# ppjian19/PhoreGen

Hardware: AMD Instinct MI355X
Metric: denoise-steps/sec (batch=128, ~40-atom graphs) (higher is better)
Workload: dtype f32; 1 GPU; BASELINE.json configs[2]: ONE batch of 128 LigPhore-shaped graphs (n~N(40,6) atoms, p~N(107,30) pharmacophore nodes), partitioned over 1 GPU(s) by the fitted step cost, steps t=999.. of the 1000-step sampler, device Philox noise, trajectory written; graphs_total=128, graphs_rank0=128, n_ctx=18401, n_lig=5115, e_knn=588832, e_bond=203720, e3=8087028, parallelism=graph-sharded x1, final RCCL gather only, triplet_workgroups_rank0=256

## Files before the change

include/phoregen_hip.h:

```cpp
#ifndef PHOREGEN_HIP_H
#define PHOREGEN_HIP_H

#include <stdint.h>

#ifdef __cplusplus
extern "C" {
#endif

const char* pg_last_error(void);
int pg_abi_version(void);
int pg_abi_struct_sizes(int* out, int n);

int pg_order_point_create(void** ev);
int pg_order_point_destroy(void* ev);
int pg_order_point_record(void* ev, void* stream);
int pg_order_point_wait(void* ev, void* stream);
int pg_debug_order_point_fence_free(int on);

enum {
  PG_OP_RECORD = 0, PG_OP_WAIT = 1, PG_OP_GEMM = 2, PG_OP_SEG_ATTN = 3, PG_OP_EMBED_CTX = 4, PG_OP_EMBED_BOND = 5, PG_OP_KNN_CTX = 6,
  PG_OP_LIG_NORMALS = 7, PG_OP_EDGE_GATE = 8, PG_OP_KNN_GROUP_BY_KIND = 9, PG_OP_BOND_SMEAR = 10, PG_OP_ATTN_FOLD_QUERY = 11,
  PG_OP_ATTN_UNFOLD_VALUE = 12, PG_OP_APPLY_DX = 13, PG_OP_LAYER_GEOM = 14, PG_OP_ROWS_LINEAR = 15, PG_OP_ATOM_COUNT = 16
};
#define PG_PROGRAM_LANES 4
#define PG_LAUNCH_MAX_ARGS 12
typedef struct {
  int32_t op;
  int32_t lane;
  int32_t ev;
  int32_t n_arg;
  uint64_t a[PG_LAUNCH_MAX_ARGS];
} PgLaunch;
int pg_program_create(const PgLaunch* list, int n, int n_events, void** prog);
int pg_program_run(void* prog, void* const* streams );
int pg_program_length(void* prog);
int pg_program_destroy(void* prog);

int pg_micro_mfma_f32(int workgroups, int iters, float* sink, double* flops, void* stream);

int pg_selftest_mfma(int* d_result, void* stream);
int pg_selftest_philox(const uint32_t* ctr_key, int n, uint32_t* out, void* stream);
int pg_debug_force_generic_seg(int mask);

typedef struct {
  const float* X;   int ldx;  int K1;
  const float* X2;  int ldx2; int K2;
  const float* W;   int ldw;
  const float* bias;
  const float* ln_gamma; const float* ln_beta;
  const float* add1; int ld_add1; const int* idx1;
  const float* add2; int ld_add2; const int* idx2;
  float out_scale;
  int   act;
  float* Y; int ldy; int M; int N;
  const int* rows;
  int add_rows;
} PgGemm;
int pg_gemm(const PgGemm* p, void* stream);
int pg_debug_gemm_streaming(int on);

typedef struct {
  int n_graphs, n_ctx, n_lig, n_phore, n_bond;
  int max_nlig;
  int max_gctx;
  const int* g_ctx_off;
  const int* g_nph;
  const int* g_nlig;
  const int* g_eid_off;
  const int* eid;
  const int* ctx_graph;
  const uint8_t* ctx_is_lig;
  const int* lig2ctx;
  const int* bond_src;
  const int* bond_dst;
  const int* bond_desc;
  const int* g_bond_off;
  const int* edge_ref;
} PgTopo;

int pg_embed_ctx(const PgTopo* t, const float* h_node_pert , const float* pos_pert ,
                 const int64_t* time_step , const float* W_node ,
                 const float* t_offset , const float* t_coeff ,
                 const float* h_phore_emb , const float* pos_phore ,
                 const int* phore2ctx , float* h_ctx , float* x_ctx ,
                 void* stream);
int pg_embed_bond(const PgTopo* t, const float* h_edge_pert , const int* bond_graph,
                  const int64_t* time_step, const float* W_edge , const float* t_offset,
                  const float* t_coeff, float* h_bond , void* stream);

// ... 187 lines not shown
```

phoregen_amd/csrc/gemm.hip:

```cpp
#include <stdlib.h>

#include "common.h"
#include "../../include/phoregen_hip.h"

namespace pg {

constexpr int BM = 128, BN = 128, BK = 32, LDT = BK + 1;


__global__ __launch_bounds__(256) void gemm_kernel(PgGemm p PG_ABL_PARAM) {
  __shared__ __attribute__((aligned(16))) float smem[(BM + BN) * LDT];
  float* const As = smem;
  float* const Bs = smem + BM * LDT;
  __shared__ float rstat[BM * 2];

  const int tid = threadIdx.x, lane = tid & 63, wave = tid >> 6;
  const int col0 = blockIdx.x * BN;
  const int K = p.K1 + p.K2;
  for (int rb = blockIdx.y; rb * BM < p.M; rb += gridDim.y) {
  const int row0 = rb * BM;
  const int wr = (wave >> 1) * 64, wc = (wave & 1) * 64;
  const bool ln = p.ln_gamma != nullptr;

  if (ln) {
// ... 187 lines not shown
  const float bias = (b && m < n_out) ? b[m] : 0.f;
  const int n_tiles = (M + 63) >> 6;
  for (int tile = blockIdx.x; tile < n_tiles; tile += gridDim.x) {
    const int row0 = tile * 64;
    __syncthreads();
#pragma unroll
    for (int i = 0; i < 8; ++i) {
      const int r = (tid >> 5) + 8 * i, c4 = tid & 31;
      int grow = row0 + r;
      grow = grow < M ? grow : M - 1;
      const int src = rows ? rows[grow] : grow;
      *reinterpret_cast<f4*>(xs + r * RL_LD + 4 * c4) = __builtin_nontemporal_load(reinterpret_cast<const f4*>(X + (size_t)src * ldx) + c4);
    }
    __syncthreads();
    f4 acc = {bias, bias, bias, bias};
    const float* xa = xs + (16 * wave + m) * RL_LD + g;
#pragma unroll
    for (int s_ = 0; s_ < 32; ++s_) acc = mfma16(xa[4 * s_], wr[s_], acc);
    if (m < n_out) {
#pragma unroll
      for (int r = 0; r < 4; ++r) {
        const int grow = row0 + 16 * wave + 4 * g + r;
        if (grow < M) Y[(size_t)grow * ldy + m] = acc[r];
      }
    }
  }
}

}

namespace pg {
bool gemm_stream_eligible(const PgGemm* p);
int launch_gemm_stream(const PgGemm* p, hipStream_t st);
}

static int g_gemm_stream = 1;
extern "C" int pg_debug_gemm_streaming(int on) { const int old = g_gemm_stream; g_gemm_stream = on; return old; }

extern "C" int pg_gemm(const PgGemm* p, void* stream) {
  if (!p || !p->X || !p->W || !p->Y || p->M < 0 || p->N <= 0) { pg::set_error("pg_gemm: bad arguments"); return PG_ERR_ARG; }
  if (p->M == 0) return PG_OK;
  if (p->K2 > 0 && !p->X2) { pg::set_error("pg_gemm: K2 > 0 without X2"); return PG_ERR_ARG; }
  if (p->ln_gamma && (p->K2 != 0 || p->K1 != 128 || (p->ldx & 3) || ((size_t)p->X & 15))) { pg::set_error("pg_gemm: LayerNorm-on-load needs K1 == 128, K2 == 0, 16-byte aligned rows"); return PG_ERR_ARG; }
  if (g_gemm_stream && pg::gemm_stream_eligible(p)) return pg::launch_gemm_stream(p, (hipStream_t)stream);
  const int row_blocks = (p->M + pg::BM - 1) / pg::BM;
  dim3 grid((p->N + pg::BN - 1) / pg::BN, row_blocks < 65535 ? row_blocks : 65535);
  hipLaunchKernelGGL(pg::gemm_kernel, grid, dim3(256), 0, (hipStream_t)stream, *p PG_ABL_ARG("PG_GEMM_ABLATE"));
  return pg::check_launch("pg_gemm");
}

extern "C" int pg_rows_linear(const float* X, int ldx, int K, const float* W, const float* b, int n_out, int M,
                              const int* rows, float* Y, int ldy, void* stream) {
  if (n_out > 16 || n_out <= 0 || K <= 0 || K > 256) { pg::set_error("pg_rows_linear: n_out must be 1..16, K 1..256"); return PG_ERR_ARG; }
  if (M == 0) return PG_OK;
  if (K == 128 && (ldx & 3) == 0 && ((size_t)X & 15) == 0) {
    int blocks = (M + 63) / 64;
    if (blocks > 8 * kNumCU) blocks = 8 * kNumCU;
    hipLaunchKernelGGL(pg::rows_linear_mfma_kernel, dim3(blocks), dim3(256), 0, (hipStream_t)stream, X, ldx, W, b, n_out, M, rows, Y, ldy);
    return pg::check_launch("pg_rows_linear");
  }
  hipLaunchKernelGGL(pg::rows_linear_kernel, dim3((M + 3) / 4), dim3(256), 0, (hipStream_t)stream, X, ldx, K, W, b,
                     n_out, M, rows, Y, ldy);
  return pg::check_launch("pg_rows_linear");
}
```

phoregen_amd/engine.py:

```python
import ctypes as C

import torch

from . import hip, options
from .packing import HEAD_SCALE, ModelPack


_SIDE_STREAMS = {}


_TRI_GRID_CACHE = {}


def side_streams(device_index, stream_set=0):
    key = (device_index, stream_set)
    if key not in _SIDE_STREAMS:
        with torch.cuda.device(device_index):
            _SIDE_STREAMS[key] = [torch.cuda.Stream(), torch.cuda.Stream(), torch.cuda.Stream()]
    return _SIDE_STREAMS[key]


def _f(*shape, device, zero=False):
    return (torch.zeros if zero else torch.empty)(*shape, dtype=torch.float32, device=device)

# ... 2 lines not shown
    __slots__ = ('kind', '__name__', 'ops', 'start', 'lane', 'tensors')

    def __init__(self, kind, name, ops=None, start=None, lane=0, tensors=()):
        self.kind, self.__name__, self.ops, self.start, self.lane, self.tensors = kind, name, ops, start, lane, tensors

    @property
    def name(self):
        return self.__name__


class Engine:
    def __init__(self, pack: ModelPack, plan, knn_k=32, full=True, phore_only=False):
        self.lib = hip.lib()
        self.pack, self.plan, self.k = pack, plan, knn_k
        self.dev = plan.device
        self._keep = []
        self.debug = None
        self.timers = None
        self.trace = None
        self.tri_calls = []
        o = options.snapshot()
        self.multi_stream = o['streams']
        self.layer_ahead = o['layer_ahead']
        self.tri_split, self.tri_split_from = o['tri_split'], o['tri_split_from']
        self.tri_overlap = o['tri_overlap']
        self.chain_q_from = o['chain_q_from']
        self.tune_grid = o['tune_grid']
        self.tuned_tri_grid = None
        self.geom_split = o['geom_split'] == 'always' or (o['geom_split'] == 'auto' and self.plan.n_bond < o['geom_split_below'])
        self.ahead_v2 = o['ahead_v2'] == 'always' or (o['ahead_v2'] == 'auto' and self.plan.n_bond < o['ahead_v2_below'])
        self.step_ahead = o['step_ahead']
        self.pos_tiled, self.pos_tiled_below = o['pos_tiled'], o['pos_tiled_below']
        self.tri_grid = o['tri_grid']
        self._lane = 0
        self._n_points = 0
        self._points = {}
        self.c_program = o['c_program']
        self._compiled = {}
        self._side = None
        self.stream_set = 0
        self._alloc()
        if full:
            self.prog_phore = self._build_phore_program()
            if not phore_only:
                self.prog_fwd = self._build_forward_program()
                self.prog_step = self.prog_ahead = None

    def _alloc(self):
        p, d = self.plan, self.dev
        n, E, k = p.n_ctx, p.n_bond, self.k
        w = self.ws = type('WS', (), {})()
        w.in_h_node, w.in_pos = _f(p.n_lig, 12, device=d), _f(p.n_lig, 3, device=d)
        w.in_h_edge = _f(E, 6, device=d)
        w.in_t = torch.zeros(p.n_graphs, dtype=torch.int64, device=d)
        w.in_t_next = torch.zeros(p.n_graphs, dtype=torch.int64, device=d)
        w.h_phore_ctx, w.x_phore_ctx = _f(n, 18, device=d, zero=True), _f(n, 3, device=d, zero=True)
        w.pos_phore, w.phore_norm = _f(p.n_phore, 3, device=d), _f(p.n_phore, 3, device=d)
        w.nrm_phore_ctx = _f(n, 3, device=d, zero=True)
        w.is_ex = torch.zeros(p.n_phore, dtype=torch.uint8, device=d)
        w.hp_ctx, w.Yp = _f(n, 128, device=d), _f(n, 640, device=d)
        w.enc_ctx = _f(n, 128, device=d, zero=True)
        w.hp_emb = _f(p.n_phore, 128, device=d)
        w.cnt_hid = _f(n, 256, device=d)
        w.s_all, w.s_l = _f(p.n_phore, device=d), _f(p.n_phore, device=d)
        w.count_l, w.count_u = _f(p.n_graphs, device=d), _f(p.n_graphs, device=d)
        w.h = [_f(n, 128, device=d), _f(n, 128, device=d)]
        w.h_in = _f(n, 128, device=d)
        w.x = [_f(n, 3, device=d), _f(n, 3, device=d)]
        w.hb = [_f(E, 128, device=d), _f(E, 128, device=d)]
        w.nbr = torch.zeros(n, k, dtype=torch.int32, device=d)
        w.deg = torch.zeros(n, dtype=torch.int32, device=d)
        w.ew, w.nrm, w.G = _f(n, k, device=d), _f(n, 3, device=d), _f(E, 20, device=d)
        w.Y1, w.Y2 = _f(n, 1920, device=d), _f(n, 1280, device=d)
        w.Y1b = None
        w.q = [_f(n, 128, device=d) for _ in range(4)]
        w.U, w.S = [_f(n, 2048, device=d) for _ in range(3)], [_f(n, 2048, device=d) for _ in range(3)]
        w.swn = [_f(n, 16, device=d) for _ in range(3)]
        w.aggE, w.aggB = _f(n, 128, device=d, zero=True), _f(n, 128, device=d, zero=True)
        w.lin_tmp = _f(n, 128, device=d)
        w.CsB, w.P = _f(E, 256, device=d), _f(E, 256, device=d)
        w.CsB2 = _f(E, 256, device=d)
        w.Qd = _f(E, 256, device=d)
        w.qhid, w.qT = _f(E, 128, device=d), _f(E, 128, device=d)
        w.dxe, w.dxb = _f(n, 3, device=d, zero=True), _f(n, 3, device=d, zero=True)
        w.head = _f(n, 128, device=d)
        w.head_b = _f(E, 128, device=d)
        w.out_v, w.out_bond = _f(p.n_lig, 12, device=d), _f(E, 6, device=d)

    def _call(self, prog, fn, *args):
        assert len(args) + 1 == len(fn.argtypes), (fn.__name__, len(args) + 1, len(fn.argtypes))
        prog.append((fn, args, self._lane if self.multi_stream else 0))

    def _new_point(self):
        self._n_points += 1
        return self._n_points - 1

    def _order(self, prog, name, ops):
        if self.multi_stream and ops:
            prog.append((_Tap('order', name, ops=ops), None, -1))

    def _fork(self, prog, lanes):
        if not self.multi_stream:
            return
        pt = self._new_point()
        self._order(prog, 'fork', [('record', pt, 0)] + [('wait', pt, l) for l in lanes])

    def _join(self, prog, lanes):
        self._sync(prog, 0, lanes, name='join')

    def _sync(self, prog, waiter, on, name='sync'):
        if not self.multi_stream:
            return
        ops = []
        for l in on:
            pt = self._new_point()
            ops += [('record', pt, l), ('wait', pt, waiter)]
# ... 11 lines not shown
            return
        self._order(prog, 'wait', [('wait', pt, waiter)])

    def _event(self, prog, name, start):
        prog.append((_Tap('event', name, start=start, lane=self._lane if self.multi_stream else 0), None, -1))

    def _mark(self, prog, name, *tensors, lane=0):
        prog.append((_Tap('mark', name, tensors=tensors, lane=lane if self.multi_stream else 0), None, -1))

    def _tap(self, tap, streams):
        if tap.kind == 'order':
            for what, pt, lane in tap.ops:
                ev = self._points.get(pt)
                if ev is None:
                    ev = self._points[pt] = hip.OrderPoint()
                if what == 'record':
                    ev.record(streams[lane])
                else:
                    ev.wait(streams[lane])
        elif tap.kind == 'event':
            if self.timers is not None:
                ev = torch.cuda.Event(enable_timing=True)
                ev.record(streams[tap.lane])
                self.timers.setdefault(tap.name, []).append((tap.start, ev))
        elif self.debug is not None:
            with torch.cuda.stream(streams[tap.lane]):
                self.debug[tap.name] = tuple(t.clone() for t in tap.tensors)

    def kernel_ms(self, name):
        evs = self.timers.get(name, [])
        return [a.elapsed_time(b) for (sa, a), (sb, b) in zip(evs[0::2], evs[1::2]) if sa and not sb]

    def _gemm(self, prog, X, K1, W, Y, M, N, bias=None, X2=None, K2=0, ln=None, add1=None, idx1=None, add2=None,
              idx2=None, scale=1.0, act=hip.ACT_NONE, rows=None):
        g = hip.PgGemm()
        g.X, g.ldx, g.K1 = X.data_ptr(), X.stride(0), K1
        g.X2, g.ldx2, g.K2 = (X2.data_ptr(), X2.stride(0), K2) if X2 is not None else (None, 0, 0)
        g.W, g.ldw = W.data_ptr(), W.stride(0)
        g.bias = hip.ptr(bias)
        g.ln_gamma, g.ln_beta = (ln[0].data_ptr(), ln[1].data_ptr()) if ln is not None else (None, None)
        g.add1, g.ld_add1, g.idx1 = (add1.data_ptr(), add1.stride(0), hip.ptr(idx1)) if add1 is not None else (None, 0, None)
        g.add2, g.ld_add2, g.idx2 = (add2.data_ptr(), add2.stride(0), hip.ptr(idx2)) if add2 is not None else (None, 0, None)
        g.out_scale, g.act = scale, act
        g.Y, g.ldy, g.M, g.N = Y.data_ptr(), Y.stride(0), M, N
        g.rows = hip.ptr(rows)
        g.add_rows = add1.size(0) if add1 is not None else 0
        self._keep += [g, X, W, Y, bias, X2, ln, add1, idx1, add2, idx2, rows]
        self._call(prog, self.lib.pg_gemm, C.byref(g))

    def _seg(self, prog, mode, n_seg, seg_ids, a, **kw):
        s = hip.PgSegAttn()
        s.mode, s.n_seg, s.seg_ids = mode, n_seg, hip.ptr(seg_ids)
        s.knn_k = self.k
        s.ln_gk, s.ln_bk, s.ln_gv, s.ln_bv = (t.data_ptr() for t in (a.ln_gk, a.ln_bk, a.ln_gv, a.ln_bv))
        for key, val in kw.items():
            setattr(s, key, val.data_ptr() if torch.is_tensor(val) else val)
            self._keep.append(val)
        self._keep += [s, seg_ids, a]
        self._call(prog, self.lib.pg_seg_attn, self.plan.topo_ref, C.byref(s))

    def _query_gemm(self, prog, a, Y, col0, h_dst_lists, buf):
        n, wq = self.plan.n_ctx, self.ws.q[buf]
        qh = Y[:, col0 + 4 * 128: col0 + 5 * 128]
        self._gemm(prog, qh, 128, a.W2q, wq, n, 128, bias=a.b2q, ln=(a.q_ln_g, a.q_ln_b), scale=HEAD_SCALE)

    def _node_attention(self, prog, mode, a, Y, col0, x, h_dst_lists, out=None, dx=None, csrc=None, buf=0, extra=None,
                        query_done=False, qbuf=None):
        w, p, n = self.ws, self.plan, self.plan.n_ctx
        wq, wU, wS, wsw = w.q[buf if qbuf is None else qbuf], w.U[buf], w.S[buf], w.swn[buf]
        blk = lambda b: Y[:, col0 + 128 * b: col0 + 128 * (b + 1)]
        if not query_done:
            self._query_gemm(prog, a, Y, col0, h_dst_lists, buf)
        knn = mode in (hip.SEG_KNN_NODE, hip.SEG_KNN_POS)
        pos = mode in (hip.SEG_KNN_POS, hip.SEG_BOND_POS)
        fused = mode != hip.SEG_PHORE
        merged = knn and len(h_dst_lists) == 2 and all(n > 0 for _, n, _ in h_dst_lists)
        lists = [h_dst_lists[0]] if merged else h_dst_lists
        for seg_ids, n_seg, is_lig in lists:
            if not fused:
                self._call(prog, self.lib.pg_attn_fold_query, wq.data_ptr(), 128, a.W2k_l.data_ptr(), n_seg,
                           seg_ids.data_ptr(), wU.data_ptr())
            kw = dict(x=x, Cdst_k=blk(0), Cdst_v=blk(1), ld_cdst=Y.stride(0), U=wU)
            if knn:
                kw.update(nrm=w.nrm, nbr=w.nbr, deg=w.deg, ew=w.ew, Csrc_k=blk(2), Csrc_v=blk(3), ld_csrc=Y.stride(0),
                          Wf_k=a.Wf_k[is_lig], Wf_v=a.Wf_v[is_lig])
                if merged:
                    ids2, n2, lig2 = h_dst_lists[1]
                    kw.update(seg_ids2=ids2, n_seg2=n2, Wf_k2=a.Wf_k[lig2], Wf_v2=a.Wf_v[lig2])
            elif mode == hip.SEG_PHORE:
                kw.update(Csrc_k=blk(2), Csrc_v=blk(3), ld_csrc=Y.stride(0), Wf_k=a.Wf_k, Wf_v=a.Wf_v)
            else:
                kw.update(Csrc_k=csrc[:, 0:128], Csrc_v=csrc[:, 128:256], ld_csrc=csrc.stride(0))
            if pos:
                kw.update(W2xv_l=a.W2xv_l, b2xv=a.b2xv, dx=dx, accumulate_dx=0)
                tiled = self.pos_tiled == 'always' or (self.pos_tiled == 'auto' and n_seg <= self.pos_tiled_below)
                if tiled:
                    kw.update(pos_tiled=1)
            else:
                kw.update(S=wS, swn=wsw)
            if fused:
                kw.update(q=wq, W2k_l=a.W2k_l)
                if not pos:
# ... 77 lines not shown
        lig = [(p.lig2ctx, p.n_lig, True)]
        both = [(p.lig2ctx, p.n_lig, True), (p.phore2ctx, p.n_phore, False)]
        L0 = pk.layers[0]
        self._sync(prog, 3, (2,))
        self._lane = 3
        self._embed_bond(prog, w.in_t_next)
        hb_done = self._record(prog, 3)
        self._lane = 2
        self._embed_ctx(prog, w.in_t_next, coords=False)
        self._first_layer_gemm(prog, L0, w.h_in, w.Y1)
        y1_done = self._record(prog, 2)
        self._query_gemm(prog, L0.NE, w.Y1, 0, both, 3)
        self._wait(prog, 2, hb_done)
        self._triplet_queries(prog, L0, w.hb[0], w.Y1)
        self._lane = 3
        self._wait(prog, 3, y1_done)
        self._bond_node_rows(prog, L0, w.hb[0], w.Y1)
        self._node_attention(prog, hip.SEG_BOND_NODE, L0.NB, w.Y1, 5 * 128, w.x[0], lig, out=w.aggB, csrc=w.CsB2, buf=2)
        self._lane = 0
        return prog

    def pipelined_programs(self):
        if not (self.step_ahead and self.multi_stream and self.layer_ahead and self.plan.n_tri_iters):
            return None
        if self.prog_step is None:
            tri_calls, self.tri_calls = self.tri_calls, []
            self.prog_step = self._build_forward_program(step_ahead=True)
            self.step_tri_calls, self.tri_calls = self.tri_calls, tri_calls
            self.prog_ahead = self._build_ahead_program()
        return self.prog_step, self.prog_ahead

    def _first_layer_gemm(self, prog, L, h_in, Y1):
        p, n = self.plan, self.plan.n_ctx
        self._gemm(prog, h_in, 128, L.W_node1, Y1, n, 1920, bias=L.b_node1)

    def _triplet_queries(self, prog, L, hb_in, Y1):
        w, p, E = self.ws, self.plan, self.plan.n_bond
        self._gemm(prog, hb_in, 128, L.TB.W_q_hb, w.qhid, E, 128, add1=Y1[:, 14 * 128:15 * 128], idx1=p.bond_dst)
        self._gemm(prog, w.qhid, 128, L.TB.W2q, w.qT, E, 128, bias=L.TB.b2q, ln=(L.TB.q_ln_g, L.TB.q_ln_b), scale=HEAD_SCALE)

    def _bond_node_rows(self, prog, L, hb_in, Y1):
        w, p, E = self.ws, self.plan, self.plan.n_bond
        self._gemm(prog, hb_in, 128, L.NB.W_hb, w.CsB2, E, 256, add1=Y1[:, 7 * 128:9 * 128], idx1=p.bond_src)

    def _denoiser_program(self, prog, lig, both, heads=None, pre_join=None, step_ahead=False):
        w, p, pk, lib = self.ws, self.plan, self.pack, self.lib
        n, E, t = p.n_ctx, p.n_bond, p.topo_ref
        h, x, hb = w.h, w.x, w.hb
        g = pk.gate
        self._fork(prog, (1,))
        self._lane = 1
        self._call(prog, lib.pg_knn_ctx, t, x[0].data_ptr(), self.k, w.nbr.data_ptr(), w.deg.data_ptr())
        self._call(prog, lib.pg_edge_gate, t, x[0].data_ptr(), w.nbr.data_ptr(), w.deg.data_ptr(), self.k,
                   g['W0'].data_ptr(), g['b0'].data_ptr(), g['g'].data_ptr(), g['b'].data_ptr(), g['W3'].data_ptr(),
                   C.c_float(g['b3']), w.ew.data_ptr())
        self._mark(prog, 'graph', w.nbr, w.deg, w.ew, lane=1)
        self._call(prog, lib.pg_knn_group_by_kind, t, self.k, w.nbr.data_ptr(), w.deg.data_ptr(), w.ew.data_ptr())
        self._lane = 0
        cur = 0
        staged = bool(p.n_tri_iters)
        n_layers = len(pk.layers)
        ahead = self.layer_ahead and self.multi_stream
        v2 = self.ahead_v2 and ahead
        chain_q = self.multi_stream and (v2 or E >= self.chain_q_from)
        tri_grid = self.tri_grid if self.tri_grid >= 0 else ((192 if E < 15000 else 224 if E < 80000 else 0) if self.multi_stream else 0)
        self._tune = None
        if (self.tune_grid and self.tri_grid < 0 and self.multi_stream and staged and 0 < tri_grid <= 224):
            self._tune = dict(cands=[g for g in (tri_grid, tri_grid + 32, tri_grid - 32) if 128 <= g <= 256])

        if v2 and w.Y1b is None:
            w.Y1b = torch.empty_like(w.Y1)
        split = v2 and self.geom_split
# ... 79 lines not shown
            self._event(prog, 'triplet', False)
            if last:
                self._fork(prog, (3,))
                self._lane = 3
                heads[0](hbn)
            self._lane = 3 if v2 else 2
            if not pre:
                bond_node_rows(L, hbc, Y1c)
                self._node_attention(prog, hip.SEG_BOND_NODE, L.NB, Y1c, 5 * 128, xc, lig, out=w.aggB, csrc=w.CsB2, buf=1)
                if v2:
                    bn_done = self._record(prog, 3)
            self._lane = 1
            if not pre:
                self._query_gemm(prog, L.NE, Y1c, 0, both, 0)
            if pre0:
                self._sync(prog, 1, (2,))
            elif pre and v2:
                self._wait(prog, 1, ne_done)
            self._event(prog, 'knn_node', True)
            self._node_attention(prog, hip.SEG_KNN_NODE, L.NE, Y1c, 0, xc1, both, out=w.aggE, buf=0, query_done=True,
                                 qbuf=3 if pre else None)
            self._event(prog, 'knn_node', False)
            if pre0:
                self._sync(prog, 1, (3,))
            elif pre or v2:
                self._wait(prog, 1, bn_done)
            else:
                self._sync(prog, 1, (2,))
            self._gemm(prog, w.aggE, 128, L.W_lin2[:, :128], w.lin_tmp, n, 128, bias=L.b_lin, add1=hc)
            self._gemm(prog, w.aggB, 128, L.W_lin2[:, 128:], hn, n, 128, add1=w.lin_tmp)
            self._mark(prog, f'A{li}', w.aggE, w.aggB, lane=1)
            if early:
                hn_done = self._record(prog, 1)
            self._gemm(prog, hn, 128, L.W_node2, w.Y2, n, 1280, bias=L.b_node2)
            if v2:
                self._query_gemm(prog, L.PB, w.Y2, 5 * 128, lig, 1)
            more_ahead = ahead and li + 1 < n_layers and not last
            self._sync(prog, 0, (1,))
            if v2 and more_ahead:
                self._lane = 1
                first_layer_gemm(pk.layers[li + 1], hn, Y1n)
                y1_done = self._record(prog, 1)
            qlane = 2 if last else 3
            if early:
                self._wait(prog, 2, hn_done)
                self._lane = 2
                heads[1](hn)
                if not v2:
                    self._fork(prog, (2,))
            else:
                self._fork(prog, (2, 3) if (ahead and li + 1 < n_layers) else (qlane,))
            self._lane = qlane
            if not v2:
                self._query_gemm(prog, L.PB, w.Y2, 5 * 128, lig, 1)
                q_done = self._record(prog, qlane)
            if last and not early:
                heads[1](hn)
            elif ahead and li + 1 < n_layers:
                Ln = pk.layers[li + 1]
                self._lane = 2
                if v2:
                    self._wait(prog, 2, y1_done)
                else:
                    first_layer_gemm(Ln, hn, Y1n)
                    y1_done = self._record(prog, 2)
                triplet_queries(Ln, hbn, Y1n)
                if not v2:
# ... 270 lines not shown
```

phoregen_amd/hip.py:

```python
import ctypes as C
import struct
import sys
import os

import torch

_HERE = os.path.dirname(os.path.abspath(__file__))
LIB_PATH = os.path.join(_HERE, '_lib', 'libphoregen_hip.so')

c_fp = C.c_void_p
c_ip = C.c_void_p


class PgGemm(C.Structure):
    _fields_ = [('X', c_fp), ('ldx', C.c_int), ('K1', C.c_int),
                ('X2', c_fp), ('ldx2', C.c_int), ('K2', C.c_int),
                ('W', c_fp), ('ldw', C.c_int),
                ('bias', c_fp),
                ('ln_gamma', c_fp), ('ln_beta', c_fp),
                ('add1', c_fp), ('ld_add1', C.c_int), ('idx1', c_ip),
                ('add2', c_fp), ('ld_add2', C.c_int), ('idx2', c_ip),
                ('out_scale', C.c_float), ('act', C.c_int),
                ('Y', c_fp), ('ldy', C.c_int), ('M', C.c_int), ('N', C.c_int), ('rows', c_ip), ('add_rows', C.c_int)]


class PgTopo(C.Structure):
    _fields_ = [('n_graphs', C.c_int), ('n_ctx', C.c_int), ('n_lig', C.c_int), ('n_phore', C.c_int),
                ('n_bond', C.c_int), ('max_nlig', C.c_int), ('max_gctx', C.c_int),
                ('g_ctx_off', c_ip), ('g_nph', c_ip), ('g_nlig', c_ip), ('g_eid_off', c_ip), ('eid', c_ip),
                ('ctx_graph', c_ip), ('ctx_is_lig', c_ip), ('lig2ctx', c_ip), ('bond_src', c_ip),
                ('bond_dst', c_ip), ('bond_desc', c_ip), ('g_bond_off', c_ip), ('edge_ref', c_ip)]


class PgSegAttn(C.Structure):
    _fields_ = [('mode', C.c_int), ('n_seg', C.c_int), ('seg_ids', c_ip), ('seg_chunks', c_ip),
                ('x', c_fp), ('nrm', c_fp), ('nbr', c_ip), ('deg', c_ip), ('ew', c_fp), ('knn_k', C.c_int),
                ('Csrc_k', c_fp), ('Csrc_v', c_fp), ('ld_csrc', C.c_int),
                ('Cdst_k', c_fp), ('Cdst_v', c_fp), ('ld_cdst', C.c_int),
                ('Wf_k', c_fp), ('Wf_v', c_fp), ('Wg2_k', c_fp), ('Wg2_v', c_fp), ('G', c_fp),
                ('ln_gk', c_fp), ('ln_bk', c_fp), ('ln_gv', c_fp), ('ln_bv', c_fp),
                ('U', c_fp), ('q', c_fp), ('W2k_l', c_fp), ('W2v_l', c_fp), ('b2v', c_fp),
                ('W2xv_l', c_fp), ('b2xv', c_fp),
                ('S', c_fp), ('swn', c_fp), ('resid', c_fp), ('out', c_fp), ('dx', c_fp),
                ('accumulate_dx', C.c_int), ('alpha', c_fp), ('alpha_rows', C.c_int), ('efeat', c_fp), ('efeat_off', c_ip),
                ('tri_iters', c_ip), ('n_tri_iters', C.c_int), ('tri_counter', c_ip),
                ('seg_ids2', c_ip), ('n_seg2', C.c_int), ('Wf_k2', c_fp), ('Wf_v2', c_fp), ('tri_grid', C.c_int), ('pos_tiled', C.c_int), ('tri_max_nlig', C.c_int)]


class PgSegAttnGrad(C.Structure):
    _fields_ = [('gS', c_fp), ('gswn', c_fp), ('gdx', c_fp), ('gU', c_fp),
                ('gCdst_k', c_fp), ('gCdst_v', c_fp), ('ld_gcdst', C.c_int),
                ('gCsrc_k', c_fp), ('gCsrc_v', c_fp), ('ld_gcsrc', C.c_int),
                ('gWf_k', c_fp), ('gWf_v', c_fp), ('gbk', c_fp), ('gbv', c_fp),
                ('gW2xv_l', c_fp), ('gb2xv', c_fp), ('gx', c_fp), ('gnrm', c_fp), ('gew', c_fp),
                ('alpha', c_fp), ('alpha_rows', C.c_int), ('S', c_fp), ('swn', c_fp),
                ('rowbuf', c_fp), ('rowbuf_rows', C.c_int), ('grid', C.c_int), ('atom_order', c_ip),
# ... 220 lines not shown
```

phoregen_amd/options.py:

```python
import contextlib
import os

DEFAULTS = dict(
    streams=True,
    layer_ahead=True,
    ahead_v2='auto',
    ahead_v2_below=82000,
    pos_tiled='auto',
    pos_tiled_below=1500,
    step_ahead=True,
    c_program=True,
    geom_split='auto',
    geom_split_below=16000,
    tune_grid=True,
    chain_q_from=150000,
    tri_split=True,
    tri_split_from=82000,
    tri_overlap=3,
    tri_grid=-1,
    dgrad_mm=True,
    rows_sum=True,
    tri_onepass=True,
    wide_gemm=True,
    bwd_atom_sort=True,
    bwd_split='all',
    bwd_grid=256,
    tri_bwd_form=2,
    tri_bwd_grid=256,
    ph_onepass=True,
)

_tri = lambda v: {'0': 'never', '1': 'auto', '2': 'always'}[v]
_flag = lambda v: v != '0'
_ENV = {
    'PG_STREAMS': ('streams', _flag),
    'PG_LAYER_AHEAD': ('layer_ahead', _flag), 'PG_AHEAD_V2': ('ahead_v2', _tri), 'PG_AHEAD_V2_BELOW': ('ahead_v2_below', int), 'PG_TRI_GRID': ('tri_grid', int), 'PG_POS_TILED': ('pos_tiled', _tri), 'PG_POS_TILED_BELOW': ('pos_tiled_below', int), 'PG_C_PROGRAM': ('c_program', _flag), 'PG_STEP_AHEAD': ('step_ahead', _flag), 'PG_CHAIN_Q_FROM': ('chain_q_from', int), 'PG_TRI_SPLIT': ('tri_split', _flag), 'PG_TUNE_GRID': ('tune_grid', _flag), 'PG_GEOM_SPLIT': ('geom_split', _tri),
    'PG_DGRAD_MM': ('dgrad_mm', _flag),
    'PG_ROWS_SUM': ('rows_sum', _flag), 'PG_TRI_ONEPASS': ('tri_onepass', _flag), 'PG_WIDE_GEMM': ('wide_gemm', _flag), 'PG_BWD_GRID': ('bwd_grid', int), 'PG_BWD_SPLIT': ('bwd_split', lambda v: {'0': 'none', '1': 'knn', '2': 'all'}[v]), 'PG_BWD_ATOM_SORT': ('bwd_atom_sort', _flag),
    'PG_TRI_BWD_FORM': ('tri_bwd_form', int), 'PG_TRI_BWD_GRID': ('tri_bwd_grid', int), 'PG_PH_ONEPASS': ('ph_onepass', _flag),
}
_overrides = {}


def get(name):
    if name in _overrides:
        return _overrides[name]
    if os.environ.get('PHOREGEN_DEBUG') == '1':
        for var, (key, conv) in _ENV.items():
            if key == name and var in os.environ:
                return conv(os.environ[var])
    return DEFAULTS[name]


def snapshot():
    return {k: get(k) for k in DEFAULTS}


@contextlib.contextmanager
def override(**kw):
    unknown = set(kw) - set(DEFAULTS)
    if unknown:
        raise KeyError(f'phoregen_amd.options: unknown switch(es) {sorted(unknown)}')
    old = dict(_overrides)
    _overrides.update(kw)
    try:
        yield
    finally:
        _overrides.clear()
        _overrides.update(old)
# ... 1 lines not shown
```

Before: 54.51 steps/s.

## Fuse attention query LayerNorm and projection into the wide node GEMM

```diff
diff --git a/include/phoregen_hip.h b/include/phoregen_hip.h
--- a/include/phoregen_hip.h
+++ b/include/phoregen_hip.h
@@ -41,6 +41,15 @@
 int pg_selftest_mfma(int* d_result, void* stream);
 int pg_selftest_philox(const uint32_t* ctr_key, int n, uint32_t* out, void* stream);
 int pg_debug_force_generic_seg(int mask);
+
+typedef struct {
+  int col0;
+  const float* ln_gamma; const float* ln_beta;
+  const float* W2; int ldw2; const float* b2;
+  float scale;
+  float* Q; int ldq;
+} PgGemmTail;
+#define PG_GEMM_MAX_TAILS 2
 
 typedef struct {
   const float* X;   int ldx;  int K1;
@@ -55,6 +64,8 @@
   float* Y; int ldy; int M; int N;
   const int* rows;
   int add_rows;
+  int n_tail;
+  PgGemmTail tail[PG_GEMM_MAX_TAILS];
 } PgGemm;
 int pg_gemm(const PgGemm* p, void* stream);
 int pg_debug_gemm_streaming(int on);
diff --git a/phoregen_amd/csrc/gemm.hip b/phoregen_amd/csrc/gemm.hip
--- a/phoregen_amd/csrc/gemm.hip
+++ b/phoregen_amd/csrc/gemm.hip
@@ -243,6 +243,8 @@
 namespace pg {
 bool gemm_stream_eligible(const PgGemm* p);
 int launch_gemm_stream(const PgGemm* p, hipStream_t st);
+const char* gemm_stream_q_refusal(const PgGemm* p);
+int launch_gemm_stream_q(const PgGemm* p, hipStream_t st);
 }
 
 static int g_gemm_stream = 1;
@@ -252,6 +254,10 @@
   if (!p || !p->X || !p->W || !p->Y || p->M < 0 || p->N <= 0) { pg::set_error("pg_gemm: bad arguments"); return PG_ERR_ARG; }
   if (p->M == 0) return PG_OK;
   if (p->K2 > 0 && !p->X2) { pg::set_error("pg_gemm: K2 > 0 without X2"); return PG_ERR_ARG; }
+  if (p->n_tail != 0) {
+    if (const char* why = pg::gemm_stream_q_refusal(p)) { pg::set_error("pg_gemm: query tail refused: %s", why); return PG_ERR_ARG; }
+    return pg::launch_gemm_stream_q(p, (hipStream_t)stream);
+  }
   if (p->ln_gamma && (p->K2 != 0 || p->K1 != 128 || (p->ldx & 3) || ((size_t)p->X & 15))) { pg::set_error("pg_gemm: LayerNorm-on-load needs K1 == 128, K2 == 0, 16-byte aligned rows"); return PG_ERR_ARG; }
   if (g_gemm_stream && pg::gemm_stream_eligible(p)) return pg::launch_gemm_stream(p, (hipStream_t)stream);
   const int row_blocks = (p->M + pg::BM - 1) / pg::BM;
diff --git a/phoregen_amd/csrc/gemm_stream_q.hip b/phoregen_amd/csrc/gemm_stream_q.hip
--- /dev/null
+++ b/phoregen_amd/csrc/gemm_stream_q.hip
@@ -0,0 +1,294 @@
+#include <type_traits>
+
+#include "wave_prims.h"
+#include "../../include/phoregen_hip.h"
+
+namespace pg {
+
+constexpr int SQ_BM = 64;
+constexpr int SQ_STAGE = SQ_BM * 128 * 4;
+
+struct SqGrid { int n_tiles, n_cb, wg_plain, wg_query; };
+
+template <int NADD >
+__global__ __launch_bounds__(256, 2) void gemm_stream_q_kernel(PgGemm p, SqGrid gr) {
+  extern __shared__ __attribute__((aligned(1024))) char st_lds[];
+  const int lane = threadIdx.x & 63;
+  const int wave = __builtin_amdgcn_readfirstlane(threadIdx.x >> 6);
+  const int l31 = lane & 31, kh = lane >> 5;
+
+  int cb = 0, first = (int)blockIdx.x, step = 1, qi = -1;
+  for (; cb < gr.n_cb; ++cb) {
+    qi = -1;
+    for (int t = 0; t < p.n_tail; ++t) if (p.tail[t].col0 == cb * 128) qi = t;
+    step = qi >= 0 ? gr.wg_query : gr.wg_plain;
+    if (first < step) break;
+    first -= step;
+  }
+  const bool isq = qi >= 0;
+  const PgGemmTail tl = qi == 1 ? p.tail[1] : p.tail[0];
+  const int colw = cb * 128 + 32 * wave;
+  const int col = colw + l31;
+
+  float Wr[64], W2r[64];
+  {
+    const float* wrow = p.W + (size_t)col * p.ldw + 4 * kh;
+#pragma unroll
+    for (int c = 0; c < 16; ++c) {
+      const f4 w = *reinterpret_cast<const f4*>(wrow + 8 * c);
+#pragma unroll
+      for (int e = 0; e < 4; ++e) Wr[4 * c + e] = w[e];
+    }
+  }
+#pragma unroll
+  for (int e = 0; e < 64; ++e) W2r[e] = 0.f;
+  float bias2 = 0.f;
+  if (isq) {
+    const float* wrow = tl.W2 + (size_t)(32 * wave + l31) * tl.ldw2 + 4 * kh;
+#pragma unroll
+    for (int c = 0; c < 16; ++c) {
+      const f4 w = *reinterpret_cast<const f4*>(wrow + 8 * c);
+#pragma unroll
+      for (int e = 0; e < 4; ++e) W2r[4 * c + e] = w[e];
+    }
+    if (tl.b2) bias2 = tl.b2[32 * wave + l31];
+  }
+  const float bias = p.bias ? p.bias[col] : 0.f;
+  f16v biasv, bias2v;
+#pragma unroll
+  for (int r = 0; r < 16; ++r) { biasv[r] = bias; bias2v[r] = bias2; }
+
+  const f4* const lnt = reinterpret_cast<const f4*>(st_lds + 2 * SQ_STAGE);
+  if (isq) {
+    float* t = reinterpret_cast<float*>(st_lds + 2 * SQ_STAGE);
+    if (threadIdx.x < 128) { t[threadIdx.x] = tl.ln_gamma[threadIdx.x]; t[128 + threadIdx.x] = tl.ln_beta[threadIdx.x]; }
+  }
+  __syncthreads();
+
+  const unsigned ldxb = (unsigned)p.ldx * 4u;
+  const unsigned ldyb = isq ? (unsigned)tl.ldq * 4u : (unsigned)p.ldy * 4u;
+  const i4v descX = raw_buffer_desc(p.X, (unsigned)p.M * ldxb);
+  const __amdgpu_buffer_rsrc_t descY = __builtin_amdgcn_make_buffer_rsrc(isq ? tl.Q : p.Y, 0, (unsigned)p.M * ldyb, 0x00020000);
+  const unsigned ocolb = (isq ? 32u * wave : (unsigned)colw) * 4u;
+  const unsigned row_sub = lane >> 3, pp = lane & 7;
+  const unsigned voff_even = row_sub * ldxb + ((pp ^ ((row_sub >> 1) & 7u)) << 4);
+  const unsigned voff_odd = row_sub * ldxb + ((pp ^ ((4u + (row_sub >> 1)) & 7u)) << 4);
+  unsigned rd[4];
+#pragma unroll
+  for (int q = 0; q < 4; ++q)
+    rd[q] = (unsigned)(l31 >> 3) * 4096u + (unsigned)(l31 & 7) * 128u + (((unsigned)(2 * q + kh) ^ ((unsigned)(l31 >> 1) & 7u)) << 4);
+  unsigned voffY[4];
+#pragma unroll
+  for (int t = 0; t < 4; ++t) voffY[t] = (unsigned)(4 * kh + t) * ldyb + (unsigned)l31 * 4u;
+  unsigned wr[2][4];
+#pragma unroll
+  for (int qo = 0; qo < 2; ++qo)
+#pragma unroll
+    for (int t = 0; t < 4; ++t)
+      wr[qo][t] = (unsigned)qo * 4096u + (unsigned)wave * 1024u + (unsigned)(4 * kh + t) * 128u +
+                  ((((unsigned)l31 >> 2) ^ (unsigned)(4 * qo + 2 * kh + (t >> 1))) << 4) + ((unsigned)l31 & 3u) * 4u;
+
+  f16v g1[2];
+  const __amdgpu_buffer_rsrc_t descI1 = __builtin_amdgcn_make_buffer_rsrc(const_cast<int*>(NADD ? p.idx1 : nullptr), 0, (unsigned)p.M * 4u, 0x00020000);
+  const __amdgpu_buffer_rsrc_t descA1 = __builtin_amdgcn_make_buffer_rsrc(const_cast<float*>(NADD ? p.add1 : nullptr), 0, 0xfffffff0u, 0x00020000);
+  const unsigned ld1b = (unsigned)p.ld_add1 * 4u;
+  const unsigned colb = (unsigned)col * 4u;
+  const unsigned last_row0 = (unsigned)p.M - SQ_BM;
+  auto tile_row0 = [&](unsigned t) { const unsigned r = t * SQ_BM; return r < last_row0 ? r : last_row0; };
+  auto load_idx = [&](unsigned row0, i4v (&ix)[8]) {
+#pragma unroll
+    for (int e = 0; e < 8; ++e) ix[e] = __builtin_amdgcn_raw_buffer_load_b128(descI1, 16u * kh, (row0 + 8u * e) * 4u, 0);
+  };
+  auto gather = [&](const i4v (&ix)[8], f16v (&g)[2]) {
+#pragma unroll
+    for (int b = 0; b < 2; ++b)
+#pragma unroll
+      for (int q = 0; q < 4; ++q)
+#pragma unroll
+        for (int t = 0; t < 4; ++t)
+          g[b][4 * q + t] = __builtin_bit_cast(
+              float, __builtin_amdgcn_raw_buffer_load_b32(descA1, (unsigned)ix[4 * b + q][t] * ld1b + colb, 0, 0));
+  };
+
+  const unsigned tile_step = (unsigned)step;
+  unsigned tile = (unsigned)first;
+  const int n_tiles = gr.n_tiles;
+
+  auto dma_tile = [&](unsigned t, unsigned stage) {
+    const unsigned row0b = tile_row0(t) * ldxb;
+#pragma unroll
+    for (int q = 0; q < 8; ++q) {
+      const unsigned i = 2u * wave + (q >> 2), j = q & 3;
+      lds_dma_1k(stage * SQ_STAGE + (i * 4u + j) * 1024u, (q >> 2) ? voff_odd : voff_even, descX, row0b + i * 8u * ldxb + j * 128u);
+    }
+  };
+
+  dma_tile(tile, 0);
+  if constexpr (NADD == 1) { i4v ix[8]; load_idx(tile_row0(tile), ix); gather(ix, g1); }
+
+  auto body = [&](auto stage_c, auto first_c) {
+    constexpr unsigned stage = decltype(stage_c)::value;
+    constexpr bool first_tile = decltype(first_c)::value;
+    if constexpr (first_tile) asm volatile("s_waitcnt vmcnt(0)\n\ts_barrier" ::: "memory");
+    else asm volatile("s_waitcnt vmcnt(32)\n\ts_barrier" ::: "memory");
+    const unsigned next = tile + tile_step;
+    dma_tile(next, stage ^ 1u);
+
+    auto frag = [&](int c, int b) {
+      return *reinterpret_cast<const f4*>(st_lds + rd[c & 3] + (stage * SQ_STAGE + b * 16384u + (c >> 2) * 1024u));
+    };
+    auto product = [&](const float (&Wv)[64], f16v (&acc)[2]) {
+      f4 aA0 = frag(0, 0), aA1 = frag(0, 1), aB0, aB1;
+#pragma unroll
+      for (int c = 0; c < 16; c += 2) {
+        aB0 = frag(c + 1, 0); aB1 = frag(c + 1, 1);
+        __builtin_amdgcn_sched_barrier(0);
+#pragma unroll
+        for (int e = 0; e < 4; ++e) {
+          acc[0] = mfma32(aA0[e], Wv[4 * c + e], acc[0]);
+          acc[1] = mfma32(aA1[e], Wv[4 * c + e], acc[1]);
+        }
+        if (c + 2 < 16) { aA0 = frag(c + 2, 0); aA1 = frag(c + 2, 1); }
+        __builtin_amdgcn_sched_barrier(0);
+#pragma unroll
+        for (int e = 0; e < 4; ++e) {
+          acc[0] = mfma32(aB0[e], Wv[4 * c + 4 + e], acc[0]);
+          acc[1] = mfma32(aB1[e], Wv[4 * c + 4 + e], acc[1]);
+        }
+      }
+      __builtin_amdgcn_sched_barrier(0);
+    };
+
+    f16v acc[2];
+    if constexpr (NADD == 1) {
+#pragma unroll
+      for (int b = 0; b < 2; ++b)
+#pragma unroll
+        for (int r = 0; r < 16; ++r) acc[b][r] = g1[b][r] + bias;
+    } else {
+      acc[0] = biasv;
+      acc[1] = biasv;
+    }
+    product(Wr, acc);
+
+    if (isq) {
+      asm volatile("s_barrier" ::: "memory");
+      char* const sb = st_lds + stage * SQ_STAGE;
+#pragma unroll
+      for (int b = 0; b < 2; ++b)
+#pragma unroll
+        for (int r = 0; r < 16; ++r)
+          *reinterpret_cast<float*>(sb + wr[(r >> 2) & 1][r & 3] + (unsigned)(b * 16384 + (r >> 3) * 8192)) = acc[b][r];
+      asm volatile("s_waitcnt lgkmcnt(0)\n\ts_barrier" ::: "memory");
+      {
+        const unsigned row = threadIdx.x >> 2, jj = threadIdx.x & 3;
+        char* const base = sb + ((row >> 3) * 4u + jj) * 1024u + (row & 7u) * 128u;
+        const unsigned sw = (row >> 1) & 7u;
+        f4 v[8];
+#pragma unroll
+        for (int q = 0; q < 8; ++q) v[q] = *reinterpret_cast<const f4*>(base + 16 * (q ^ sw));
+        float sm = 0.f;
+#pragma unroll
+        for (int q = 0; q < 8; ++q) sm += (v[q][0] + v[q][1]) + (v[q][2] + v[q][3]);
+        sm += __shfl_xor(sm, 1);
+        sm += __shfl_xor(sm, 2);
+        const float mu = sm * (1.f / 128.f);
+        float qs = 0.f;
+#pragma unroll
+        for (int q = 0; q < 8; ++q)
+#pragma unroll
+          for (int e = 0; e < 4; ++e) { const float d = v[q][e] - mu; qs = fmaf(d, d, qs); }
+        qs += __shfl_xor(qs, 1);
+        qs += __shfl_xor(qs, 2);
+        const float rs = 1.0f / sqrtf(qs * (1.f / 128.f) + 1e-5f);
+#pragma unroll
+        for (int q = 0; q < 8; ++q) {
+          const unsigned k4 = 8u * jj + (unsigned)q;
+          const f4 ga = lnt[k4], be = lnt[32 + k4];
+          f4 o;
+#pragma unroll
+          for (int e = 0; e < 4; ++e) o[e] = fmaxf((v[q][e] - mu) * rs * ga[e] + be[e], 0.f);
+          *reinterpret_cast<f4*>(base + 16 * (q ^ sw)) = o;
+        }
+      }
+      asm volatile("s_waitcnt lgkmcnt(0)\n\ts_barrier" ::: "memory");
+      acc[0] = bias2v;
+      acc[1] = bias2v;
+      product(W2r, acc);
+#pragma unroll
+      for (int b = 0; b < 2; ++b)
+#pragma unroll
+        for (int r = 0; r < 16; ++r) acc[b][r] *= tl.scale;
+    }
+
+    const unsigned row0 = tile_row0(tile);
+#pragma unroll
+    for (int b = 0; b < 2; ++b)
+#pragma unroll
+      for (int r = 0; r < 16; ++r) {
+        const unsigned soff = (row0 + 32u * b + 8u * (r >> 2)) * ldyb + ocolb;
+        const float v = acc[b][r];
+        __builtin_amdgcn_raw_buffer_store_b32(__builtin_bit_cast(int, v), descY, voffY[r & 3], soff, 0);
+      }
+    if constexpr (NADD == 1) { i4v ix1[8]; load_idx(tile_row0(next), ix1); gather(ix1, g1); }
+    tile = next;
+  };
+
+  if ((int)tile < n_tiles) {
+    body(std::integral_constant<unsigned, 0>{}, std::true_type{});
+    while ((int)tile < n_tiles) {
+      body(std::integral_constant<unsigned, 1>{}, std::false_type{});
+      if ((int)tile >= n_tiles) break;
+      body(std::integral_constant<unsigned, 0>{}, std::false_type{});
+    }
+  }
+  asm volatile("s_waitcnt vmcnt(0)" ::: "memory");
+}
+
+constexpr float SQ_QUERY_WEIGHT = 2.25f;
+
+template <int NADD>
+static int launch_stream_q_t(const PgGemm* p, hipStream_t st) {
+  const void* k = reinterpret_cast<const void*>(gemm_stream_q_kernel<NADD>);
+  const size_t lds = 2 * SQ_STAGE + 1024;
+  if (int rc = reserve_lds(k, lds, "pg_gemm(stream, query tail)")) return rc;
+  SqGrid gr;
+  gr.n_tiles = (p->M + SQ_BM - 1) / SQ_BM;
+  gr.n_cb = p->N / 128;
+  const int n_plain = gr.n_cb - p->n_tail;
+  const float unit = 2.f * kNumCU / ((float)n_plain + SQ_QUERY_WEIGHT * p->n_tail);
+  gr.wg_plain = (int)unit;
+  gr.wg_query = (int)(unit * SQ_QUERY_WEIGHT);
+  if (gr.wg_plain < 1) gr.wg_plain = 1;
+  if (gr.wg_query < 1) gr.wg_query = 1;
+  if (gr.wg_plain > gr.n_tiles) gr.wg_plain = gr.n_tiles;
+  if (gr.wg_query > gr.n_tiles) gr.wg_query = gr.n_tiles;
+  const int grid = n_plain * gr.wg_plain + p->n_tail * gr.wg_query;
+  hipLaunchKernelGGL((gemm_stream_q_kernel<NADD>), dim3(grid), dim3(256), lds, st, *p, gr);
+  return check_launch("pg_gemm(stream, query tail)");
+}
+
+const char* gemm_stream_q_refusal(const PgGemm* p) {
+  if (p->n_tail < 0 || p->n_tail > PG_GEMM_MAX_TAILS) return "n_tail out of range";
+  if (p->K1 != 128 || p->K2 != 0 || p->rows || p->act != 0 || p->ln_gamma || p->out_scale != 1.0f || p->add2) return "not the plain K = 128 streaming shape";
+  if ((p->N & 127) || p->M < SQ_BM) return "N must be a multiple of 128 and M at least 64";
+  if ((p->ldx & 3) || ((size_t)p->X & 15) || (p->ldw & 3) || ((size_t)p->W & 15)) return "X and W rows must be 16-byte aligned";
+  if (p->add1 && !p->idx1) return "the added operand must be gathered (idx1)";
+  if (p->add1 && (p->add_rows <= 0 || (size_t)p->add_rows * p->ld_add1 * 4 >= 0xfffff000ull)) return "add_rows missing or the added operand too large";
+  if ((size_t)p->M * p->ldx * 4 >= 0xfffff000ull || (size_t)p->M * p->ldy * 4 >= 0xfffff000ull) return "X or Y too large for 32-bit offsets";
+  for (int t = 0; t < p->n_tail; ++t) {
+    const PgGemmTail& q = p->tail[t];
+    if (q.col0 < 0 || (q.col0 & 127) || q.col0 >= p->N) return "tail col0 must be a multiple of 128 below N";
+    if (t && q.col0 == p->tail[0].col0) return "two tails on one column block";
+    if (!q.ln_gamma || !q.ln_beta || !q.W2 || !q.Q) return "tail pointer missing";
+    if ((q.ldw2 & 3) || ((size_t)q.W2 & 15)) return "tail W2 rows must be 16-byte aligned";
+    if (q.ldq < 128 || (size_t)p->M * q.ldq * 4 >= 0xfffff000ull) return "tail Q rows too short or too large for 32-bit offsets";
+  }
+  return nullptr;
+}
+
+int launch_gemm_stream_q(const PgGemm* p, hipStream_t st) {
+  return p->add1 ? launch_stream_q_t<1>(p, st) : launch_stream_q_t<0>(p, st);
+}
+
+}
diff --git a/phoregen_amd/engine.py b/phoregen_amd/engine.py
--- a/phoregen_amd/engine.py
+++ b/phoregen_amd/engine.py
@@ -58,6 +58,9 @@
         self.step_ahead = o['step_ahead']
         self.pos_tiled, self.pos_tiled_below = o['pos_tiled'], o['pos_tiled_below']
         self.tri_grid = o['tri_grid']
+        fq = o['fused_query'] if plan.n_ctx >= 64 else 'none'
+        self.fuse_node_q = fq in ('node', 'all')
+        self.fuse_bond_q = fq == 'all' and plan.n_bond >= 64
         self._lane = 0
         self._n_points = 0
         self._points = {}
@@ -108,6 +111,7 @@
         w.CsB2 = _f(E, 256, device=d)
         w.Qd = _f(E, 256, device=d)
         w.qhid, w.qT = _f(E, 128, device=d), _f(E, 128, device=d)
+        w.qf = {}
         w.dxe, w.dxb = _f(n, 3, device=d, zero=True), _f(n, 3, device=d, zero=True)
         w.head = _f(n, 128, device=d)
         w.head_b = _f(E, 128, device=d)
@@ -185,7 +189,7 @@
         return [a.elapsed_time(b) for (sa, a), (sb, b) in zip(evs[0::2], evs[1::2]) if sa and not sb]
 
     def _gemm(self, prog, X, K1, W, Y, M, N, bias=None, X2=None, K2=0, ln=None, add1=None, idx1=None, add2=None,
-              idx2=None, scale=1.0, act=hip.ACT_NONE, rows=None):
+              idx2=None, scale=1.0, act=hip.ACT_NONE, rows=None, tails=()):
         g = hip.PgGemm()
         g.X, g.ldx, g.K1 = X.data_ptr(), X.stride(0), K1
         g.X2, g.ldx2, g.K2 = (X2.data_ptr(), X2.stride(0), K2) if X2 is not None else (None, 0, 0)
@@ -198,6 +202,12 @@
         g.Y, g.ldy, g.M, g.N = Y.data_ptr(), Y.stride(0), M, N
         g.rows = hip.ptr(rows)
         g.add_rows = add1.size(0) if add1 is not None else 0
+        g.n_tail = len(tails)
+        for tl, (col0, a, Q) in zip(g.tail, tails):
+            tl.col0, tl.ln_gamma, tl.ln_beta = col0, a.q_ln_g.data_ptr(), a.q_ln_b.data_ptr()
+            tl.W2, tl.ldw2, tl.b2, tl.scale = a.W2q.data_ptr(), a.W2q.stride(0), a.b2q.data_ptr(), HEAD_SCALE
+            tl.Q, tl.ldq = Q.data_ptr(), Q.stride(0)
+            self._keep += [a, Q]
         self._keep += [g, X, W, Y, bias, X2, ln, add1, idx1, add2, idx2, rows]
         self._call(prog, self.lib.pg_gemm, C.byref(g))
 
@@ -212,7 +222,21 @@
         self._keep += [s, seg_ids, a]
         self._call(prog, self.lib.pg_seg_attn, self.plan.topo_ref, C.byref(s))
 
+    def _fused_q(self, Y, col0):
+        w = self.ws
+        if not self.fuse_node_q or not (Y is w.Y1 or Y is w.Y1b or Y is w.Y2):
+            return None
+        key = (Y.data_ptr(), col0)
+        if key not in w.qf:
+            w.qf[key] = _f(self.plan.n_ctx, 128, device=self.dev)
+        return w.qf[key]
+
+    def _node_tails(self, Y, subs):
+        return [(col0 + 4 * 128, a, self._fused_q(Y, col0)) for col0, a in subs] if self._fused_q(Y, subs[0][0]) is not None else []
+
     def _query_gemm(self, prog, a, Y, col0, h_dst_lists, buf):
+        if self._fused_q(Y, col0) is not None:
+            return
         n, wq = self.plan.n_ctx, self.ws.q[buf]
         qh = Y[:, col0 + 4 * 128: col0 + 5 * 128]
         self._gemm(prog, qh, 128, a.W2q, wq, n, 128, bias=a.b2q, ln=(a.q_ln_g, a.q_ln_b), scale=HEAD_SCALE)
@@ -221,6 +245,8 @@
                         query_done=False, qbuf=None):
         w, p, n = self.ws, self.plan, self.plan.n_ctx
         wq, wU, wS, wsw = w.q[buf if qbuf is None else qbuf], w.U[buf], w.S[buf], w.swn[buf]
+        if self._fused_q(Y, col0) is not None:
+            wq = self._fused_q(Y, col0)
         blk = lambda b: Y[:, col0 + 128 * b: col0 + 128 * (b + 1)]
         if not query_done:
             self._query_gemm(prog, a, Y, col0, h_dst_lists, buf)
@@ -364,12 +390,14 @@
 
     def _first_layer_gemm(self, prog, L, h_in, Y1):
         p, n = self.plan, self.plan.n_ctx
-        self._gemm(prog, h_in, 128, L.W_node1, Y1, n, 1920, bias=L.b_node1)
+        self._gemm(prog, h_in, 128, L.W_node1, Y1, n, 1920, bias=L.b_node1, tails=self._node_tails(Y1, [(0, L.NE), (5 * 128, L.NB)]))
 
     def _triplet_queries(self, prog, L, hb_in, Y1):
         w, p, E = self.ws, self.plan, self.plan.n_bond
-        self._gemm(prog, hb_in, 128, L.TB.W_q_hb, w.qhid, E, 128, add1=Y1[:, 14 * 128:15 * 128], idx1=p.bond_dst)
-        self._gemm(prog, w.qhid, 128, L.TB.W2q, w.qT, E, 128, bias=L.TB.b2q, ln=(L.TB.q_ln_g, L.TB.q_ln_b), scale=HEAD_SCALE)
+        self._gemm(prog, hb_in, 128, L.TB.W_q_hb, w.qhid, E, 128, add1=Y1[:, 14 * 128:15 * 128], idx1=p.bond_dst,
+                   tails=[(0, L.TB, w.qT)] if self.fuse_bond_q else ())
+        if not self.fuse_bond_q:
+            self._gemm(prog, w.qhid, 128, L.TB.W2q, w.qT, E, 128, bias=L.TB.b2q, ln=(L.TB.q_ln_g, L.TB.q_ln_b), scale=HEAD_SCALE)
 
     def _bond_node_rows(self, prog, L, hb_in, Y1):
         w, p, E = self.ws, self.plan, self.plan.n_bond
@@ -515,7 +543,7 @@
             self._mark(prog, f'A{li}', w.aggE, w.aggB, lane=1)
             if early:
                 hn_done = self._record(prog, 1)
-            self._gemm(prog, hn, 128, L.W_node2, w.Y2, n, 1280, bias=L.b_node2)
+            self._gemm(prog, hn, 128, L.W_node2, w.Y2, n, 1280, bias=L.b_node2, tails=self._node_tails(w.Y2, [(0, L.PE), (5 * 128, L.PB)]))
             if v2:
                 self._query_gemm(prog, L.PB, w.Y2, 5 * 128, lig, 1)
             more_ahead = ahead and li + 1 < n_layers and not last
diff --git a/phoregen_amd/hip.py b/phoregen_amd/hip.py
--- a/phoregen_amd/hip.py
+++ b/phoregen_amd/hip.py
@@ -10,6 +10,14 @@
 
 c_fp = C.c_void_p
 c_ip = C.c_void_p
+
+
+class PgGemmTail(C.Structure):
+    _fields_ = [('col0', C.c_int), ('ln_gamma', c_fp), ('ln_beta', c_fp), ('W2', c_fp), ('ldw2', C.c_int), ('b2', c_fp),
+                ('scale', C.c_float), ('Q', c_fp), ('ldq', C.c_int)]
+
+
+PG_GEMM_MAX_TAILS = 2
 
 
 class PgGemm(C.Structure):
@@ -21,7 +29,8 @@
                 ('add1', c_fp), ('ld_add1', C.c_int), ('idx1', c_ip),
                 ('add2', c_fp), ('ld_add2', C.c_int), ('idx2', c_ip),
                 ('out_scale', C.c_float), ('act', C.c_int),
-                ('Y', c_fp), ('ldy', C.c_int), ('M', C.c_int), ('N', C.c_int), ('rows', c_ip), ('add_rows', C.c_int)]
+                ('Y', c_fp), ('ldy', C.c_int), ('M', C.c_int), ('N', C.c_int), ('rows', c_ip), ('add_rows', C.c_int),
+                ('n_tail', C.c_int), ('tail', PgGemmTail * PG_GEMM_MAX_TAILS)]
 
 
 class PgTopo(C.Structure):
diff --git a/phoregen_amd/options.py b/phoregen_amd/options.py
--- a/phoregen_amd/options.py
+++ b/phoregen_amd/options.py
@@ -18,6 +18,7 @@
     tri_split_from=82000,
     tri_overlap=3,
     tri_grid=-1,
+    fused_query='node',
     dgrad_mm=True,
     rows_sum=True,
     tri_onepass=True,
@@ -34,7 +35,7 @@
 _flag = lambda v: v != '0'
 _ENV = {
     'PG_STREAMS': ('streams', _flag),
-    'PG_LAYER_AHEAD': ('layer_ahead', _flag), 'PG_AHEAD_V2': ('ahead_v2', _tri), 'PG_AHEAD_V2_BELOW': ('ahead_v2_below', int), 'PG_TRI_GRID': ('tri_grid', int), 'PG_POS_TILED': ('pos_tiled', _tri), 'PG_POS_TILED_BELOW': ('pos_tiled_below', int), 'PG_C_PROGRAM': ('c_program', _flag), 'PG_STEP_AHEAD': ('step_ahead', _flag), 'PG_CHAIN_Q_FROM': ('chain_q_from', int), 'PG_TRI_SPLIT': ('tri_split', _flag), 'PG_TUNE_GRID': ('tune_grid', _flag), 'PG_GEOM_SPLIT': ('geom_split', _tri),
+    'PG_LAYER_AHEAD': ('layer_ahead', _flag), 'PG_AHEAD_V2': ('ahead_v2', _tri), 'PG_AHEAD_V2_BELOW': ('ahead_v2_below', int), 'PG_TRI_GRID': ('tri_grid', int), 'PG_FUSED_QUERY': ('fused_query', lambda v: {'0': 'none', '1': 'node', '2': 'all'}[v]), 'PG_POS_TILED': ('pos_tiled', _tri), 'PG_POS_TILED_BELOW': ('pos_tiled_below', int), 'PG_C_PROGRAM': ('c_program', _flag), 'PG_STEP_AHEAD': ('step_ahead', _flag), 'PG_CHAIN_Q_FROM': ('chain_q_from', int), 'PG_TRI_SPLIT': ('tri_split', _flag), 'PG_TUNE_GRID': ('tune_grid', _flag), 'PG_GEOM_SPLIT': ('geom_split', _tri),
     'PG_DGRAD_MM': ('dgrad_mm', _flag),
     'PG_ROWS_SUM': ('rows_sum', _flag), 'PG_TRI_ONEPASS': ('tri_onepass', _flag), 'PG_WIDE_GEMM': ('wide_gemm', _flag), 'PG_BWD_GRID': ('bwd_grid', int), 'PG_BWD_SPLIT': ('bwd_split', lambda v: {'0': 'none', '1': 'knn', '2': 'all'}[v]), 'PG_BWD_ATOM_SORT': ('bwd_atom_sort', _flag),
     'PG_TRI_BWD_FORM': ('tri_bwd_form', int), 'PG_TRI_BWD_GRID': ('tri_bwd_grid', int), 'PG_PH_ONEPASS': ('ph_onepass', _flag),
```

Result: slower. 53.89 steps/s (-1.1%).
